# nextpyp/spr_pick

Measured on AMD Instinct MI355X. Metric: train_patches_per_sec, higher is better.
Workload: dtype f32

## Files before the change

spr_pick_amd/csrc/wino.h:

```cpp
#pragma once
#include <hip/hip_runtime.h>

#include "corr.h"

namespace sprk {

bool wino_eligible(const Corr &c);
size_t wino_ws_bytes(const Corr &c);
int wino_conv(const Corr &c, const float *x, const float *x2, const float *w, float *y, float *U, const float *mask,
              int mask_act, hipStream_t s, int unrotB = 0);
bool wino_unrot_eligible(const Corr &c);
bool wino_wgrad_eligible(const sprk_conv_geom &g);
size_t wino_wgrad_ws_bytes(const sprk_conv_geom &g);
int wino_wgrad(const sprk_conv_geom &g, const float *x, const float *x2, const float *gy, float *gw, void *ws,
               sprk_reduce_item *, hipStream_t s);

}
```

spr_pick_amd/csrc/wino.hip:

```cpp
#include <algorithm>
#include <cstdio>
#include <cstdlib>

#include "common.h"
#include "wino.h"
#include "wprep_dev.h"

namespace {

typedef float f32x4 __attribute__((ext_vector_type(4)));
typedef float f32x2 __attribute__((ext_vector_type(2)));
typedef unsigned u32x2 __attribute__((ext_vector_type(2)));
typedef unsigned u32x4 __attribute__((ext_vector_type(4)));
__device__ __forceinline__ unsigned fbits(float v) { return __builtin_bit_cast(unsigned, v); }
typedef __attribute__((address_space(3))) void lds_void;
typedef __amdgpu_buffer_rsrc_t rsrc_t;
constexpr int kXZero = (int)0x80000000;
constexpr float kLeak = 0.1f;

__device__ __forceinline__ rsrc_t make_rsrc(const void *p) {
    return __builtin_amdgcn_make_buffer_rsrc(const_cast<void *>(p), 0, 0x7FFFFFFF, 0x00020000);
}
__device__ __forceinline__ const float *uniform_ptr(const float *p) {
    const unsigned long v = (unsigned long)p;
    const unsigned lo = __builtin_amdgcn_readfirstlane((unsigned)v), hi = __builtin_amdgcn_readfirstlane((unsigned)(v >> 32));
    return (const float *)(((unsigned long)hi << 32) | lo);
}
__device__ __forceinline__ void bdma16(rsrc_t r, int voff, int soff, float *lds_wave_base) {
    __builtin_amdgcn_raw_ptr_buffer_load_lds(r, (lds_void *)lds_wave_base, 16, voff, soff, 0, 0);
}
typedef const __attribute__((address_space(3))) float *lds_cfp;
__device__ __forceinline__ int lds_addr(const void *p) {
    return (int)(unsigned)(__SIZE_TYPE__)(const __attribute__((address_space(3))) char *)p;
}
__device__ __forceinline__ lds_cfp lds_f(int byte_addr) { return (lds_cfp)(__SIZE_TYPE__)(unsigned)byte_addr; }

__device__ __forceinline__ void lds_barrier() {
    asm volatile("s_waitcnt lgkmcnt(0)" ::: "memory");
    __builtin_amdgcn_s_barrier();
    asm volatile("" ::: "memory");
}

__device__ __forceinline__ float act_fn(float v, int act) {
    if (act == SPRK_ACT_LEAKY) return v > 0.f ? v : v * kLeak;
    if (act == SPRK_ACT_RELU) return v > 0.f ? v : 0.f;
    return v;
}

constexpr int CK = sprk::kWinoCK;
template <int SQ>
struct Geo {
    static constexpr int TR = SQ ? 16 : 8, TC = SQ ? 16 : 32;
    static constexpr int RP = TC + 8, RPLANE = (TR + 2) * RP;
    static constexpr int LGTX = SQ ? 3 : 4;
};
constexpr int RAWF = 1792;
static_assert(CK * Geo<0>::RPLANE <= RAWF && CK * Geo<1>::RPLANE <= RAWF, "raw tile fits its stage");
constexpr int ETS = 68;
constexpr int kThreads = 512;
constexpr int kEFloats = 4 * 2 * 32 * ETS;
constexpr int kECFloats = 2 * 96;

__host__ __device__ constexpr int ufloats_of(int NT) { return 16 * NT * CK * 16; }
__host__ __device__ constexpr size_t lds_bytes_of(int NT) {
    return (size_t)(2 * RAWF + 2 * ufloats_of(NT) + kEFloats + kECFloats) * 4;
}

template <int V>
struct IC {
    static constexpr int value = V;
};

#ifdef WINO_STAMP
#define STAMP(k) do { __builtin_amdgcn_sched_barrier(0); if (P == 0) { unsigned long t_; asm volatile("s_memtime %0\n\ts_waitcnt lgkmcnt(0)" : "=s"(t_) :: "memory"); st[(k)] = (unsigned)t_; } __builtin_amdgcn_sched_barrier(0); } while (0)
#else
#define STAMP(k)
#endif
struct KArgs {
    const float *x, *x2, *U, *bias, *scale, *shift, *mask;
    float *y;
    int N, C1, C2, H, W, Cout, padT, padL, act, tilesX, tilesY, ntiles, nc1, nch, up2, xcd, diag, mact;
    int unrotB;
#ifdef WINO_STAMP
    unsigned *dbg;
#endif
};

template <int NT, int SQ, int UNROT = 0>
__global__ __launch_bounds__(kThreads, 1) void wino_conv_kernel(const KArgs a) {
    constexpr int UFLOATS = ufloats_of(NT);
    constexpr int TR = Geo<SQ>::TR, TC = Geo<SQ>::TC, RP = Geo<SQ>::RP, RPLANE = Geo<SQ>::RPLANE, LGTX = Geo<SQ>::LGTX;
    extern __shared__ __attribute__((aligned(16))) float smem[];
    float *Ub = smem;
    float *Rb = smem + 2 * UFLOATS;
    const int tid = threadIdx.x, lane = tid & 63, wave = __builtin_amdgcn_readfirstlane(tid >> 6), l15 = lane & 15,
              lq = lane >> 4;
    const int pg = wave & 3, th = wave >> 2;
    const int grp = blockIdx.y;
    const long HW = (long)a.H * a.W;
    float *EC = smem + 2 * UFLOATS + 2 * RAWF + kEFloats;
    if (tid < NT * 16) {
        const int co = grp * (NT * 16) + tid;
        float sc = 1.f, sh = 0.f;
        if (co < a.Cout) {
            if (a.scale) {
                sc = a.scale[co];
                sh = a.shift[co];
            } else if (a.bias) {
                sh = a.bias[co];
            }
        }
        EC[tid] = sc;
        EC[96 + tid] = sh;
    }

    constexpr int RAWQ = CK * RPLANE / 4;
    int dch = 4, lrow = 0x7000, lcol = 0, loff = 0;
    if (tid < RAWQ) {
        dch = tid / (RPLANE / 4);
        const int rem = tid % (RPLANE / 4);
        lrow = rem / (RP / 4);
        lcol = 4 * (rem % (RP / 4)) - 4;
        loff = (int)(((long)dch * a.H + lrow) * a.W + lcol + 4) * 4;
    }
    int n = 0, by = 0, bx = 0, voff = kXZero;
    auto set_tile = [&](int tile) {
        const int t0 = __builtin_amdgcn_readfirstlane(tile);
        const int q0 = __builtin_amdgcn_readfirstlane(t0 / a.tilesX);
        bx = t0 - q0 * a.tilesX;
        n = __builtin_amdgcn_readfirstlane(q0 / a.tilesY);
        by = q0 - n * a.tilesY;
        const unsigned gy = (unsigned)(by * TR - a.padT + lrow), gx = (unsigned)(bx * TC + lcol);
        voff = (gy < (unsigned)a.H && gx < (unsigned)a.W) ? loff : kXZero;
    };
    const float *rawcur = nullptr, *rawsrc2 = nullptr;
    auto raw_begin = [&]() {
        const long org = (long)(by * TR - a.padT) * a.W + bx * TC - 4;
        rawcur = uniform_ptr(a.x + (long)n * a.C1 * HW + org);
        rawsrc2 = a.C2 > 0 ? uniform_ptr(a.x2 + (long)n * a.C2 * HW + org) : nullptr;
    };
    const int rag1 = (a.C1 % CK) ? a.nc1 - 1 : -1, rag2 = (a.C2 % CK) ? a.nch - 1 : -1;
    auto issue_raw = [&](int c, float *dst, auto ragged) {
        if (c == a.nc1) rawcur = rawsrc2;
        const rsrc_t rs = make_rsrc(rawcur);
        rawcur += (long)CK * HW;
        int vo = voff;
        if constexpr (decltype(ragged)::value != 0)
            if (c == rag1 || c == rag2) vo = dch < (c == rag1 ? a.C1 % CK : a.C2 % CK) ? voff : kXZero;
        if (wave < 7) bdma16(rs, vo, 0, dst + wave * 256);
    };
    const float *Ug = a.U + (long)grp * a.nch * UFLOATS;
    auto issue_u = [&](int c, float *dst) {
        const rsrc_t ur = make_rsrc(Ug + (long)c * UFLOATS);
        constexpr int full = UFLOATS / 2048, rest = UFLOATS % 2048;
#pragma unroll
        for (int gi = 0; gi < full; ++gi) bdma16(ur, tid * 16, gi * 8192, dst + gi * 2048 + wave * 256);
        if (rest && wave < rest / 256) bdma16(ur, tid * 16, full * 8192, dst + full * 2048 + wave * 256);
    };

    f32x4 acc[4][2][NT];

    const int ra = pg == 0 ? 0 : pg == 2 ? 2 : 1, rb = pg == 3 ? 3 : pg == 2 ? 1 : 2;
    const float sgn = pg == 1 ? 1.f : -1.f;
    int rawA[2], rawB[2];
    const int trow0 = (32 * th + l15) >> LGTX, tcol0 = l15 & ((1 << LGTX) - 1);
    constexpr int MTROWS = 16 >> LGTX;
    rawA[0] = lds_addr(Rb + lq * RPLANE + (2 * trow0 + ra) * RP + (4 - a.padL) + 2 * tcol0);
    rawB[0] = lds_addr(Rb + lq * RPLANE + (2 * trow0 + rb) * RP + (4 - a.padL) + 2 * tcol0);
    rawA[1] = rawA[0] + RAWF * 4;
    rawB[1] = rawB[0] + RAWF * 4;
    int bbase = lds_addr(Ub + (4 * pg) * NT * 64 + (NT % 2 == 0 ? 2 * lane : lane));
    asm volatile("" : "+v"(rawA[0]), "+v"(rawA[1]), "+v"(rawB[0]), "+v"(rawB[1]), "+v"(bbase));

    auto transform = [&](auto stage, float (&av)[2][4]) {
        constexpr int S = decltype(stage)::value;
        const lds_cfp pa = lds_f(rawA[S]), pb = lds_f(rawB[S]);
#pragma unroll
        for (int mt = 0; mt < 2; ++mt) {
            float xv[4];
#pragma unroll
            for (int j = 0; j < 4; ++j)
                xv[j] = __builtin_fmaf(pb[mt * 2 * MTROWS * RP + j], sgn, pa[mt * 2 * MTROWS * RP + j]);
            av[mt][0] = xv[0] - xv[2];
            av[mt][1] = xv[1] + xv[2];
            av[mt][2] = xv[2] - xv[1];
            av[mt][3] = xv[1] - xv[3];
        }
    };
    auto mfma12 = [&](const float (&av)[2][4], const float (&bv)[NT], auto pos, auto first) {
        constexpr int p = decltype(pos)::value;
        constexpr bool FIRST = decltype(first)::value != 0;
#pragma unroll
        for (int mt = 0; mt < 2; ++mt)
#pragma unroll
            for (int nt = 0; nt < NT; ++nt) {
                if constexpr (FIRST)
                    acc[p][mt][nt] = __builtin_amdgcn_mfma_f32_16x16x4f32(av[mt][p], bv[nt], (f32x4){0.f, 0.f, 0.f, 0.f}, 0, 0, 0);
                else
                    acc[p][mt][nt] = __builtin_amdgcn_mfma_f32_16x16x4f32(av[mt][p], bv[nt], acc[p][mt][nt], 0, 0, 0);
            }
    };
    auto loadb = [&](float (&bv)[NT], auto stage, auto pos) {
        constexpr int S = decltype(stage)::value, p = decltype(pos)::value;
        if constexpr (NT % 2 == 0) {
            typedef const __attribute__((address_space(3))) f32x2 *lds_cf2p;
#pragma unroll
            for (int q = 0; q < NT / 2; ++q) {
                const f32x2 v = *(lds_cf2p)(__SIZE_TYPE__)(unsigned)(bbase + (S * UFLOATS + (p * (NT / 2) + q) * 128) * 4);
                bv[2 * q] = v[0];
                bv[2 * q + 1] = v[1];
            }
        } else {
            const lds_cfp bp = lds_f(bbase);
#pragma unroll
            for (int nt = 0; nt < NT; ++nt) bv[nt] = bp[S * UFLOATS + (p * NT + nt) * 64];
        }
    };

#ifdef WINO_STAMP
    unsigned st[8] = {}, sv[8] = {};
    if (NT == 6 && a.dbg && blockIdx.x < 4 && lane == 0) {
        a.dbg[(blockIdx.x * 8 + wave) * 16 + 10] = (unsigned)__builtin_amdgcn_s_memtime();
        a.dbg[(blockIdx.x * 8 + wave) * 16 + 11] = (unsigned)__builtin_amdgcn_s_memrealtime();
    }
#endif
    const int nch = a.nch;
    int tile = xcd_slot(blockIdx.x, gridDim.x, a.xcd);
    set_tile(tile);
    auto first_loads = [&]() {
        raw_begin();
        issue_raw(0, Rb, IC<1>{});
        issue_u(0, Ub);
        if (nch > 1) issue_raw(1, Rb + RAWF, IC<1>{});
    };
    first_loads();
    asm volatile("s_waitcnt vmcnt(0)" ::: "memory");
    __syncthreads();
    float aop[2][2][4];
    transform(IC<0>{}, aop[0]);
    __syncthreads();
    auto iter = [&](auto par, int c, auto first, auto checked) {
        constexpr int P = decltype(par)::value;
        constexpr bool CHK = decltype(checked)::value != 0;
        STAMP(0);
        if (!CHK || c + 1 < nch) issue_u(c + 1, Ub + (1 - P) * UFLOATS);
        if (!CHK || c + 2 < nch) issue_raw(c + 2, Rb + P * RAWF, checked);
        STAMP(1);
        float b0[NT], b1[NT];
        if constexpr (NT == 6) {
            transform(IC<1 - P>{}, aop[1 - P]);
            STAMP(2);
            loadb(b0, IC<P>{}, IC<0>{}); mfma12(aop[P], b0, IC<0>{}, first);
            STAMP(3);
            loadb(b0, IC<P>{}, IC<1>{}); mfma12(aop[P], b0, IC<1>{}, first);
            STAMP(4);
            loadb(b0, IC<P>{}, IC<2>{}); mfma12(aop[P], b0, IC<2>{}, first);
            STAMP(5);
            loadb(b0, IC<P>{}, IC<3>{}); mfma12(aop[P], b0, IC<3>{}, first);
            STAMP(6);
            (void)b1;
        } else {
            loadb(b0, IC<P>{}, IC<0>{});
            loadb(b1, IC<P>{}, IC<1>{});
            __builtin_amdgcn_sched_barrier(0);
            mfma12(aop[P], b0, IC<0>{}, first);
            __builtin_amdgcn_sched_barrier(0);
            loadb(b0, IC<P>{}, IC<2>{});
            transform(IC<1 - P>{}, aop[1 - P]);
            __builtin_amdgcn_sched_barrier(0);
            mfma12(aop[P], b1, IC<1>{}, first);
            __builtin_amdgcn_sched_barrier(0);
            loadb(b1, IC<P>{}, IC<3>{});
            __builtin_amdgcn_sched_barrier(0);
            mfma12(aop[P], b0, IC<2>{}, first);
            __builtin_amdgcn_sched_barrier(0);
            mfma12(aop[P], b1, IC<3>{}, first);
        }
        asm volatile("s_waitcnt vmcnt(0)" ::: "memory");
        STAMP(7);
        __syncthreads();
#ifdef WINO_STAMP
        if (c == 10) for (int k = 0; k < 8; ++k) sv[k] = st[k];
#endif
    };
    for (;;) {
        iter(IC<0>{}, 0, IC<1>{}, IC<1>{});
        if (1 < nch) iter(IC<1>{}, 1, IC<0>{}, IC<1>{});
        int c = 2;
        if (rag1 < 0)
            for (; c + 4 < nch; c += 2) {
                iter(IC<0>{}, c, IC<0>{}, IC<0>{});
                iter(IC<1>{}, c + 1, IC<0>{}, IC<0>{});
            }
        for (; c < nch; c += 2) {
            iter(IC<0>{}, c, IC<0>{}, IC<1>{});
            if (c + 1 < nch) iter(IC<1>{}, c + 1, IC<0>{}, IC<1>{});
        }
        const int e_n = n, e_by = by, e_bx = bx;
        const int next = tile + (int)gridDim.x;
        const bool more = next < a.ntiles;
        if (more) {
            set_tile(next);
            first_loads();
        }

    float *E = smem + 2 * UFLOATS + 2 * RAWF;
    const int rl_tx = lane & ((1 << LGTX) - 1), rl_ty = lane >> LGTX;
    int tprime = lane;
    int uoffA = kXZero, uoffB = kXZero, uoffE = kXZero, urot = 0, uk = 0, ub = 0;
    bool uzero = false;
    if constexpr (UNROT) {
        uk = __builtin_amdgcn_readfirstlane(e_n / a.unrotB);
        ub = e_n - uk * a.unrotB;
        urot = (4 - uk) & 3;
        const int P = a.W;
        const int tx = (urot & 1) ? lane >> (6 - LGTX) : rl_tx, ty = (urot & 1) ? lane & ((64 >> LGTX) - 1) : rl_ty;
        tprime = (ty << LGTX) + tx;
        const int s0 = e_by * TR + 2 * ty, v0 = e_bx * TC + 2 * tx;
        const bool top = s0 == 0, last = s0 == P - 2;
        uzero = top;
        if (urot == 0) {
            uoffA = ((s0 + 1) * P + v0) * 4;
            uoffB = last ? kXZero : uoffA + P * 4;
            uoffE = top ? v0 * 4 : kXZero;
        } else if (urot == 2) {
            uoffA = ((P - 2 - s0) * P + (P - 2 - v0)) * 4;
            uoffB = last ? kXZero : uoffA - P * 4;
            uoffE = top ? ((P - 1) * P + (P - 2 - v0)) * 4 : kXZero;
        } else if (urot == 3) {
            uoffA = last ? kXZero : (v0 * P + (P - 3 - s0)) * 4;
            uoffB = last ? kXZero : uoffA + P * 4;
            uoffE = top ? (v0 * P + P - 1) * 4 : last ? (v0 * P) * 4 : kXZero;
        } else {
            uoffA = last ? kXZero : ((P - 1 - v0) * P + s0 + 1) * 4;
            uoffB = last ? kXZero : uoffA - P * 4;
            uoffE = top ? ((P - 2 - v0) * P) * 4 : last ? ((P - 2 - v0) * P + P - 1) * 4 : kXZero;
        }
    }
    const int lane_off = a.up2 ? ((4 * rl_ty) * (2 * a.W) + 4 * rl_tx) * 4 : ((2 * rl_ty) * a.W + 2 * rl_tx) * 4;
    const long tile_org = a.up2 ? ((long)(2 * e_by * TR) * (2 * a.W) + 2 * e_bx * TC) : ((long)(e_by * TR) * a.W + e_bx * TC);
    const long plane = a.up2 ? 4 * HW : HW;
    constexpr int PASSES = (NT + 1) / 2;
    if (!(a.diag & 1))
#pragma unroll
    for (int pass = 0; pass < PASSES; ++pass) {
#pragma unroll
        for (int n2 = 0; n2 < 2; ++n2) {
            const int nt = pass * 2 + n2;
            if (nt < NT) {
#pragma unroll
                for (int mt = 0; mt < 2; ++mt) {
                    const f32x4 s0 = (acc[0][mt][nt] + acc[1][mt][nt]) + acc[2][mt][nt];
                    const f32x4 s1 = (acc[1][mt][nt] - acc[2][mt][nt]) - acc[3][mt][nt];
                    float *e = E + ((pg * 2) * 32 + n2 * 16 + l15) * ETS + 4 * lq + 16 * mt + 32 * th;
                    *reinterpret_cast<f32x4 *>(e) = s0;
                    *reinterpret_cast<f32x4 *>(e + 32 * ETS) = s1;
                }
            }
        }
        lds_barrier();
        auto reader = [&](auto modec) {
            constexpr int MODE = decltype(modec)::value;
            const long ch0 = (MODE == 3 ? (long)(ub * 4 + uk) : (long)e_n) * a.Cout + grp * (NT * 16) + pass * 32 + wave;
            const float *yc = uniform_ptr(a.y + ch0 * plane + (MODE == 3 ? 0 : tile_org));
            const float *mc = MODE == 1 ? uniform_ptr(a.mask + ch0 * plane + tile_org) : nullptr;
#pragma unroll
            for (int it = 0; it < 4; ++it) {
                const int cp = wave + 8 * it;
                const int co = grp * (NT * 16) + pass * 32 + cp;
                if (pass * 32 + cp < NT * 16 && co < a.Cout) {
                    f32x2 mk0 = {1.f, 1.f}, mk1 = {1.f, 1.f};
                    if constexpr (MODE == 1) {
                        const rsrc_t mr = make_rsrc(mc);
                        mk0 = __builtin_bit_cast(f32x2, __builtin_amdgcn_raw_buffer_load_b64(mr, lane_off, 0, 0));
                        mk1 = __builtin_bit_cast(f32x2, __builtin_amdgcn_raw_buffer_load_b64(mr, lane_off, 4 * a.W, 0));
                    }
                    f32x2 s[4];
#pragma unroll
                    for (int w = 0; w < 4; ++w) {
                        s[w][0] = E[((w * 2 + 0) * 32 + cp) * ETS + tprime];
                        s[w][1] = E[((w * 2 + 1) * 32 + cp) * ETS + tprime];
                    }
                    const float sc = EC[pass * 32 + cp], sh = EC[96 + pass * 32 + cp];
                    f32x2 o0 = ((s[0] + s[1]) + s[2]) * sc + sh;
                    f32x2 o1 = ((s[1] - s[2]) - s[3]) * sc + sh;
                    if (a.act == SPRK_ACT_LEAKY) {
                        o0 = __builtin_elementwise_max(o0, o0 * kLeak);
                        o1 = __builtin_elementwise_max(o1, o1 * kLeak);
                    } else if (a.act == SPRK_ACT_RELU) {
                        o0 = __builtin_elementwise_max(o0, (f32x2){0.f, 0.f});
                        o1 = __builtin_elementwise_max(o1, (f32x2){0.f, 0.f});
                    }
                    if constexpr (MODE == 1) {
                        const float neg = a.mact == SPRK_ACT_LEAKY ? kLeak : 0.f;
                        o0[0] *= mk0[0] > 0.f ? 1.f : neg;
                        o0[1] *= mk0[1] > 0.f ? 1.f : neg;
                        o1[0] *= mk1[0] > 0.f ? 1.f : neg;
                        o1[1] *= mk1[1] > 0.f ? 1.f : neg;
                    }
                    const rsrc_t yr = make_rsrc(yc);
                    if constexpr (MODE == 3) {
                        const int rowb = 4 * a.W;
                        if (urot & 1) {
                            const bool rev = urot == 3;
                            __builtin_amdgcn_raw_buffer_store_b64((u32x2){fbits(rev ? o1[0] : o0[0]), fbits(rev ? o0[0] : o1[0])}, yr, uoffA, 0, 0);
                            __builtin_amdgcn_raw_buffer_store_b64((u32x2){fbits(rev ? o1[1] : o0[1]), fbits(rev ? o0[1] : o1[1])}, yr, uoffB, 0, 0);
                            const unsigned e0 = uzero ? 0u : fbits(rev ? o0[0] : o0[1]), e1 = uzero ? 0u : fbits(rev ? o0[1] : o0[0]);
                            __builtin_amdgcn_raw_buffer_store_b32(e0, yr, uoffE, 0, 0);
                            __builtin_amdgcn_raw_buffer_store_b32(e1, yr, uoffE, rowb, 0);
                        } else {
                            const bool rev = urot == 2;
                            __builtin_amdgcn_raw_buffer_store_b64((u32x2){fbits(rev ? o0[1] : o0[0]), fbits(rev ? o0[0] : o0[1])}, yr, uoffA, 0, 0);
                            __builtin_amdgcn_raw_buffer_store_b64((u32x2){fbits(rev ? o1[1] : o1[0]), fbits(rev ? o1[0] : o1[1])}, yr, uoffB, 0, 0);
                            __builtin_amdgcn_raw_buffer_store_b64((u32x2){0u, 0u}, yr, uoffE, 0, 0);
                        }
                    } else if constexpr (MODE == 2) {
                        const int W2b = 8 * a.W;
                        const u32x4 r0 = {fbits(o0[0]), fbits(o0[0]), fbits(o0[1]), fbits(o0[1])},
                                    r1 = {fbits(o1[0]), fbits(o1[0]), fbits(o1[1]), fbits(o1[1])};
                        __builtin_amdgcn_raw_buffer_store_b128(r0, yr, lane_off, 0, 0);
                        __builtin_amdgcn_raw_buffer_store_b128(r0, yr, lane_off, W2b, 0);
                        __builtin_amdgcn_raw_buffer_store_b128(r1, yr, lane_off, 2 * W2b, 0);
                        __builtin_amdgcn_raw_buffer_store_b128(r1, yr, lane_off, 3 * W2b, 0);
                    } else {
                        __builtin_amdgcn_raw_buffer_store_b64((u32x2){fbits(o0[0]), fbits(o0[1])}, yr, lane_off, 0, 0);
                        __builtin_amdgcn_raw_buffer_store_b64((u32x2){fbits(o1[0]), fbits(o1[1])}, yr, lane_off, 4 * a.W, 0);
                    }
                }
                yc += 8 * plane;
                if constexpr (MODE == 1) mc += 8 * plane;
            }
        };
        if constexpr (UNROT)
            reader(IC<3>{});
        else if (a.up2)
            reader(IC<2>{});
        else if (a.mask)
            reader(IC<1>{});
        else
            reader(IC<0>{});
        lds_barrier();
    }
#ifdef WINO_STAMP
        if (NT == 6 && a.dbg && blockIdx.x < 4 && lane == 0) {
            if (tile < (int)gridDim.x) a.dbg[(blockIdx.x * 8 + wave) * 16 + 12] = (unsigned)__builtin_amdgcn_s_memtime();
            a.dbg[(blockIdx.x * 8 + wave) * 16 + 13] = (unsigned)__builtin_amdgcn_s_memtime();
            a.dbg[(blockIdx.x * 8 + wave) * 16 + 14] = (unsigned)__builtin_amdgcn_s_memrealtime();
        }
#endif
        if (!more) break;
        tile = next;
        asm volatile("s_waitcnt vmcnt(0)" ::: "memory");
        __syncthreads();
        transform(IC<0>{}, aop[0]);
        __syncthreads();
    }
}

constexpr int WRH = 4, WRW = 16, WRP = 24;
constexpr int WPB = 4 * 3 * 16 + 4;
constexpr int WAF = 4 * 2048, WSTAGE = 2 * WAF;
constexpr size_t kWgLdsBytes = (size_t)(2 * WSTAGE) * 4;

struct WgKArgs {
    const float *x, *gy;
    float *partial;
    int N, Csrc, cbase, ci0, CinTot, H, W, Cout, padT, padL, regionsX, regionsY, xcd;
};

template <int MT>
__global__ __launch_bounds__(kThreads, 1) void wino_wgrad_kernel(const WgKArgs a) {
    constexpr int PA = 6 * MT * WRP + 4, NA4 = 16 * (PA / 4), NB4 = 32 * (WPB / 4);
    static_assert(16 * PA <= WAF && 32 * WPB <= WAF, "stage holds both operands");
    extern __shared__ __attribute__((aligned(16))) float smem[];
    const int tid = threadIdx.x, lane = tid & 63, wave = __builtin_amdgcn_readfirstlane(tid >> 6), l15 = lane & 15,
              lq = lane >> 4;
    const int pg = wave & 3, h = wave >> 2;
    const int grp = blockIdx.y;
    const int H = a.H, W = a.W;
    const long HW = (long)H * W;
    const int nregions = a.N * a.regionsY * a.regionsX;
    const int c0 = a.cbase + grp * 16 * MT;
    const int have = a.Csrc - c0;

    int offA[4], offB[4], mskA[4];
    {
        const int RY = a.regionsY, RX = a.regionsX;
#pragma unroll
        for (int rd = 0; rd < 4; ++rd) {
            const int q = tid + rd * kThreads;
            const int sl = q / (PA / 4), rem = q % (PA / 4);
            const int row = rem / (6 * MT), mt = (rem % (6 * MT)) / 6, c4 = rem % 6;
            const bool va = q < NA4 && rem < 36 * MT && 16 * mt + sl < have;
            offA[rd] = va ? (int)(((16 * mt + sl) * HW + (long)row * W + 4 * c4) * 4) : kXZero;
            int m = 0;
#pragma unroll
            for (int yt = 0; yt < 4; ++yt) {
                const int ry = yt == 0 ? 0 : yt == 1 ? 1 : yt == 2 ? RY - 1 : 0;
                const bool rok = (unsigned)(ry * WRH - a.padT + row) < (unsigned)H;
#pragma unroll
                for (int xt = 0; xt < 4; ++xt) {
                    const int rx = xt == 0 ? 0 : xt == 1 ? 1 : xt == 2 ? RX - 1 : 0;
                    const bool cok = (unsigned)(rx * WRW - 4 + 4 * c4) < (unsigned)W;
                    m |= (rok && cok) ? 1 << (4 * yt + xt) : 0;
                }
            }
            mskA[rd] = va ? m : 0;
            const int sb = q / (WPB / 4), remb = q % (WPB / 4);
            const int rowb = remb / 12, ntb = (remb % 12) / 4, c4b = remb % 4;
            const int chb = (sb >> 4) * 48 + 16 * ntb + (sb & 15);
            offB[rd] = (q < NB4 && remb < 48 && chb < a.Cout) ? (int)((chb * HW + (long)rowb * W + 4 * c4b) * 4) : kXZero;
        }
    }
    int cur_rx, cur_ry, cur_n, d_rx, d_ry, d_n;
    {
        const int r0 = xcd_slot(blockIdx.x, gridDim.x, a.xcd);
        const int q0 = r0 / a.regionsX;
        cur_rx = __builtin_amdgcn_readfirstlane(r0 - q0 * a.regionsX);
        cur_n = __builtin_amdgcn_readfirstlane(q0 / a.regionsY);
        cur_ry = __builtin_amdgcn_readfirstlane(q0 - (q0 / a.regionsY) * a.regionsY);
        const int st = gridDim.x, t0 = st / a.regionsX;
        d_rx = __builtin_amdgcn_readfirstlane(st - t0 * a.regionsX);
        d_n = __builtin_amdgcn_readfirstlane(t0 / a.regionsY);
        d_ry = __builtin_amdgcn_readfirstlane(t0 - (t0 / a.regionsY) * a.regionsY);
// ... 144 lines not shown
    }
    };
    if (zmix) {
        regions(IC<1>{});
        finish();
    } else {
        regions(IC<0>{});
        finish();
    }
}

struct WgRanges {
    int end[4], parts[4];
};
__global__ __launch_bounds__(256) void wino_wgrad_reduce_kernel(const float *__restrict__ partial, float *__restrict__ gw,
                                                                long n, int CinTot, WgRanges rg) {
    __shared__ float red[8][33];
    const int el = threadIdx.x & 31, sl = threadIdx.x >> 5;
    const long e = (long)blockIdx.x * 32 + el;
    float s = 0.f;
    if (e < n) {
        const int ci = (int)((e / 9) % CinTot);
        int parts = rg.parts[3];
#pragma unroll
        for (int i = 2; i >= 0; --i)
            if (ci < rg.end[i]) parts = rg.parts[i];
        float s0 = 0.f, s1 = 0.f;
        int p = sl;
        for (; p + 8 < parts; p += 16) {
            s0 += partial[(long)p * n + e];
            s1 += partial[(long)(p + 8) * n + e];
        }
        if (p < parts) s0 += partial[(long)p * n + e];
        s = s0 + s1;
    }
    red[sl][el] = s;
    __syncthreads();
    if (sl == 0 && e < n) {
        float t = red[0][el];
#pragma unroll
        for (int j = 1; j < 8; ++j) t += red[j][el];
        gw[e] = t;
    }
}

bool wg_split(int C, int *g48, int *tail) {
    *g48 = C / 48;
    *tail = C % 48;
    return *tail <= 16;
}

int nt_of(int Cout) { return Cout <= 48 ? 3 : 6; }

int wino_square(int H, int W) {
    if (H % Geo<0>::TR == 0 && W % Geo<0>::TC == 0) return 0;
    if (H % Geo<1>::TR == 0 && W % Geo<1>::TC == 0) return 1;
    return -1;
}

}

namespace sprk {

constexpr int kClassWino = 3;

bool wino_eligible(const Corr &g) {
    static const int on = knob_env("SPRK_WINO", 1);
    if (!on) return false;
    if (g.KH != 3 || g.KW != 3 || g.stride != 1 || g.dil != 1 || g.up1 || g.mfma_only || g.ep.res) return false;
    if (g.Hout != g.Hin || g.Wout != g.Win) return false;
    const int H = g.Hin, W = g.Win;
    const int sq = wino_square(H, W);
    if (sq < 0) return false;
    const int TR = sq ? Geo<1>::TR : Geo<0>::TR, TC = sq ? Geo<1>::TC : Geo<0>::TC;
    if (g.padL < 0 || g.padL > 4 || g.padT < 0) return false;
    if (g.C1 < 1 || g.C2 < 0 || g.Cout < 33) return false;
    const int NT = nt_of(g.Cout), groups = cdiv(g.Cout, NT * 16);
    if ((double)g.Cout / (groups * NT * 16) < 0.7) return false;
    if (!g.pin() && (long)g.N * (H / TR) * (W / TC) * groups < 128) return false;
    if ((long)4 * H * W * 4 >= 0x7FFFFFFFL) return false;
    return true;
}

size_t wino_ws_bytes(const Corr &c) {
    const int NT = nt_of(c.Cout), groups = cdiv(c.Cout, NT * 16), nch = cdiv(c.C1, CK) + cdiv(c.C2, CK);
    return (size_t)groups * nch * ufloats_of(NT) * sizeof(float);
}

bool wino_unrot_eligible(const Corr &c) {
    return wino_eligible(c) && nt_of(c.Cout) == 6 && c.Hin == 64 && c.Win == 64 && c.N % 4 == 0 && !c.ep.up2 && c.taps == 0;
}

int wino_conv(const Corr &w, const float *x, const float *x2, const float *taps, float *y, float *U, const float *mask,
              int mask_act, hipStream_t s, int unrotB) {
    const int NT = nt_of(w.Cout), groups = cdiv(w.Cout, NT * 16);
    const int kclass = w.Cout > 48 ? kClassWino : 2;
    KArgs a{};
    a.x = x; a.x2 = x2; a.U = U; a.bias = w.ep.bias; a.scale = w.ep.scale; a.shift = w.ep.shift; a.y = y;
    a.N = w.N; a.C1 = w.C1; a.C2 = w.C2; a.H = w.Hin; a.W = w.Win; a.Cout = w.Cout; a.padT = w.padT; a.padL = w.padL;
    a.act = w.ep.act;
    a.up2 = w.ep.up2 ? 1 : 0;
    a.mask = a.up2 ? nullptr : mask;
    a.mact = mask_act;
    a.xcd = xcd_on();
    static const int diag = sprk::diag_env("SPRK_WINO_DIAG");
    a.diag = diag;
    a.unrotB = unrotB;
    if (unrotB && (mask || !wino_unrot_eligible(w) || unrotB * 4 != w.N)) {
        set_error("wino_conv: no un-rotated store for this call");
        return SPRK_EINVAL;
    }
    static const int unrot_sq = knob_env("SPRK_WINO_UNROT_SQ", 0);
    const int sq = (unrotB && unrot_sq) ? 1 : wino_square(a.H, a.W);
    a.tilesX = a.W / (sq ? Geo<1>::TC : Geo<0>::TC); a.tilesY = a.H / (sq ? Geo<1>::TR : Geo<0>::TR);
    a.ntiles = a.tilesX * a.tilesY * w.N;
    a.nc1 = cdiv(w.C1, CK);
    a.nch = a.nc1 + cdiv(w.C2, CK);
    if ((((uintptr_t)x | (uintptr_t)x2 | (uintptr_t)y | (uintptr_t)U) & 15) != 0) {
        set_error("wino_conv: tensors must be 16-byte aligned");
        return SPRK_EINVAL;
    }
    const long total = (long)groups * a.nch * NT * CK * 16;
    if (int rc = wprep_site(wprep_item(WPREP_WINO, taps, U, total, {w.Cout, w.C1, w.C2, a.nc1, a.nch, NT, groups, w.taps}), s))
        return rc;
    static const int persist = knob_env("SPRK_WINO_PERSIST", 1);
    const dim3 grid(persist ? std::min(a.ntiles, std::max(1, num_cus() / groups)) : a.ntiles, groups);
    const size_t lds = lds_bytes_of(NT);
    auto launch = [&](auto kernel) {
        if (int rc = lds_optin(kernel, lds, "wino_conv")) return rc;
        hipLaunchKernelGGL(kernel, grid, dim3(kThreads), lds, s, a);
        return (int)SPRK_OK;
    };
#ifdef WINO_STAMP
    static unsigned *dbg = nullptr;
    static int dumped = 0;
    if (!dbg) { hipMalloc(&dbg, 4 * 8 * 16 * 4); hipMemset(dbg, 0, 4 * 8 * 16 * 4); }
    a.dbg = dbg;
#endif
    prof_begin(kclass, w.flops, s);
    if (int rc = unrotB ? (sq ? launch(wino_conv_kernel<6, 1, 1>) : launch(wino_conv_kernel<6, 0, 1>))
                 : NT == 6 ? (sq ? launch(wino_conv_kernel<6, 1>) : launch(wino_conv_kernel<6, 0>))
                         : (sq ? launch(wino_conv_kernel<3, 1>) : launch(wino_conv_kernel<3, 0>)))
        return rc;
    prof_end(kclass, s);
#ifdef WINO_STAMP
    if (NT == 6 && !sq && ++dumped == 5 && getenv("SPRK_WINO_STAMP")) {
        hipDeviceSynchronize();
        unsigned h[4 * 8 * 16];
        hipMemcpy(h, dbg, sizeof h, hipMemcpyDeviceToHost);
        FILE *f = fopen(getenv("SPRK_WINO_STAMP"), "a");
        for (int wg = 0; wg < 4; ++wg)
            for (int wv = 0; wv < 8; ++wv) {
                fprintf(f, "wg%d w%d", wg, wv);
                for (int k = 0; k < 16; ++k) fprintf(f, " %u", h[(wg * 8 + wv) * 16 + k]);
                fprintf(f, "\n");
            }
        fclose(f);
    }
#endif
    g_wino_launches.fetch_add(1, std::memory_order_relaxed);
    return SPRK_OK;
}

bool wino_wgrad_eligible(const sprk_conv_geom &g) {
    static const int on = knob_env("SPRK_WINO_WGRAD", 1);
    if (!on) return false;
    if (g.KH != 3 || g.KW != 3 || g.stride != 1 || g.dil != 1 || g.up1) return false;
    const int H = g.Hin, W = g.Win, padT = g.pad_top, padL = g.pad_left;
    if (g.Hout != H || g.Wout != W || H % WRH || W % WRW) return false;
    if (padL < 0 || padL > 4 || padT < 0 || padT > 4) return false;
    if (g.Cout < 81 || g.Cout > 96) return false;
    int g48, tail;
    if (g.C1 < 1 || !wg_split(g.C1, &g48, &tail)) return false;
    if (g.C2 > 0 && !wg_split(g.C2, &g48, &tail)) return false;
    static const long min_regions = knob_env("SPRK_WINO_WGRAD_MIN", 0);
    const bool has_tail = (g.C1 % 48) != 0 || (g.C2 % 48) != 0;
    const long need = min_regions > 0 ? min_regions : (has_tail ? 8192 : 2048);
    if ((long)g.N * (H / WRH) * (W / WRW) < need) return false;
    if ((long)48 * H * W * 4 >= 0x7FFFFFFFL || (long)g.Cout * H * W * 4 >= 0x7FFFFFFFL) return false;
    return true;
}

constexpr int kWgParts = 256;
constexpr int kClassWinoW = 4;

size_t wino_wgrad_ws_bytes(const sprk_conv_geom &g) {
    return (size_t)kWgParts * g.Cout * (g.C1 + g.C2) * 9 * sizeof(float);
}

int wino_wgrad(const sprk_conv_geom &g, const float *x, const float *x2, const float *gy, float *gw, void *ws,
               sprk_reduce_item *, hipStream_t s) {
    float *partial = (float *)ws;
    if ((((uintptr_t)x | (uintptr_t)x2 | (uintptr_t)gy | (uintptr_t)partial) & 15) != 0) {
        set_error("wino_wgrad: tensors must be 16-byte aligned");
        return SPRK_EINVAL;
    }
    const double flops = conv_flops(g);
    const int CinTot = g.C1 + g.C2;
    WgRanges rg{};
    int nr = 0;
    auto launch = [&](const float *src, int Csrc, int ci0) -> int {
        int g48, tail;
        wg_split(Csrc, &g48, &tail);
        WgKArgs a{src, gy, partial, g.N, Csrc, 0, ci0, CinTot, g.Hin, g.Win, g.Cout, g.pad_top, g.pad_left, g.Win / WRW,
                  g.Hin / WRH, xcd_on()};
        if (g48 > 0) {
            if (int rc = lds_optin(wino_wgrad_kernel<3>, kWgLdsBytes, "wino_wgrad")) return rc;
            const int parts = std::min(kWgParts, num_cus()) / g48;
            prof_begin(kClassWinoW, flops * (48.0 * g48) / CinTot, s);
            hipLaunchKernelGGL(wino_wgrad_kernel<3>, dim3(parts, g48), dim3(kThreads), kWgLdsBytes, s, a);
            prof_end(kClassWinoW, s);
            if (int rc = check_launch("wino_wgrad<3>")) return rc;
            rg.end[nr] = ci0 + 48 * g48;
            rg.parts[nr++] = parts;
        }
        if (tail > 0) {
            if (int rc = lds_optin(wino_wgrad_kernel<1>, kWgLdsBytes, "wino_wgrad")) return rc;
            WgKArgs t = a;
            t.cbase = 48 * g48;
            prof_begin(kClassWinoW, flops * (double)tail / CinTot, s);
            hipLaunchKernelGGL(wino_wgrad_kernel<1>, dim3(std::min(kWgParts, num_cus()), 1), dim3(kThreads), kWgLdsBytes, s, t);
            prof_end(kClassWinoW, s);
            if (int rc = check_launch("wino_wgrad<1>")) return rc;
            rg.end[nr] = ci0 + Csrc;
            rg.parts[nr++] = std::min(kWgParts, num_cus());
        }
        return SPRK_OK;
    };
    if (int rc = launch(x, g.C1, 0)) return rc;
    if (g.C2 > 0)
        if (int rc = launch(x2, g.C2, g.C1)) return rc;
    for (int i = nr; i < 4; ++i) rg.end[i] = CinTot, rg.parts[i] = rg.parts[nr - 1];
    const long n = (long)g.Cout * CinTot * 9;
    hipLaunchKernelGGL(wino_wgrad_reduce_kernel, dim3(cdiv(n, 32)), dim3(256), 0, s, partial, gw, n, CinTot, rg);
    if (int rc = check_launch("wino_wgrad_reduce")) return rc;
    g_wino_launches.fetch_add(1, std::memory_order_relaxed);
    return SPRK_OK;
}

}
```

Measured before the change: 1981.

## Specialize Winograd epilogue by form and share buffer descriptors across channels

The output epilogue of the Winograd conv kernel is restructured into compile-time specialized variants keyed by a host-computed form code that covers store mode, activation/affine kind and shared-descriptor use. This removes per-channel runtime activation branches and buffer resource rebuilds. When the planes fit in the 32-bit buffer range, a single descriptor is reused with a scalar channel offset. Tile index decode also switches from per-tile divisions to incremental advancement, and the inverse-transform adds are split into half-vectors. Each form becomes its own specialized copy of the epilogue, which increases code size and adds a dispatch switch; a new ISA counting script is also added.

After: 1979. No clear change (-0.1%).

```diff
diff --git a/profiles/isa_count.py b/profiles/isa_count.py
--- /dev/null
+++ b/profiles/isa_count.py
@@ -0,0 +1,104 @@
+#!/usr/bin/env python3
+import argparse
+import re
+import sys
+
+CLASSES = ["mfma", "valu", "pk", "scalar", "lds_rd", "lds_wr", "buf_ld", "buf_st", "wait", "barrier", "other"]
+
+
+def classify(m):
+    if m.startswith(("v_mfma", "v_smfmac")):
+        return "mfma"
+    if m.startswith("v_pk_"):
+        return "pk"
+    if m.startswith("v_"):
+        return "valu"
+    if m.startswith("s_waitcnt"):
+        return "wait"
+    if m.startswith("s_barrier"):
+        return "barrier"
+    if m.startswith("s_"):
+        return "scalar"
+    if m.startswith(("ds_read", "ds_load")):
+        return "lds_rd"
+    if m.startswith(("ds_write", "ds_store")):
+        return "lds_wr"
+    if m.startswith("buffer_load"):
+        return "buf_ld"
+    if m.startswith("buffer_store"):
+        return "buf_st"
+    return "other"
+
+
+LABEL = re.compile(r"^([A-Za-z_.$][\w.$]*):")
+INSN = re.compile(r"^\s+([a-z][a-z0-9_]*)\b(.*)$")
+
+
+def kernels(lines):
+    names = [m.group(1) for ln in lines if (m := re.match(r"^\s*\.amdhsa_kernel\s+(\S+)", ln))]
+    out = {}
+    for name in names:
+        start = next((i for i, ln in enumerate(lines) if ln.startswith(name + ":")), None)
+        if start is None:
+            continue
+        end = next((i for i in range(start, len(lines)) if lines[i].startswith(".Lfunc_end")), len(lines))
+        out[name] = (start + 1, end)
+    return out
+
+
+def blocks(lines, lo, hi):
+    out = [("<entry>", dict.fromkeys(CLASSES, 0), [])]
+    for ln in lines[lo:hi]:
+        code = ln.split(";")[0].rstrip()
+        if not code:
+            continue
+        if m := LABEL.match(code):
+            out.append((m.group(1), dict.fromkeys(CLASSES, 0), []))
+            continue
+        m = INSN.match(code)
+        if not m or code.lstrip().startswith("."):
+            continue
+        mnem, rest = m.group(1), m.group(2)
+        out[-1][1][classify(mnem)] += 1
+        if mnem.startswith(("s_cbranch", "s_branch", "s_endpgm", "s_setpc")):
+            out[-1][2].append(rest.strip())
+            base, _, k = out[-1][0].partition("+")
+            out.append(("%s+%d" % (base, int(k or 0) + 1), dict.fromkeys(CLASSES, 0), []))
+    return out
+
+
+def main():
+    ap = argparse.ArgumentParser(description=__doc__, formatter_class=argparse.RawDescriptionHelpFormatter)
+    ap.add_argument("asm", help="assembly of one source (hipcc ... --cuda-device-only -S)")
+    ap.add_argument("kernel", nargs="?", help="substring of the kernel's symbol")
+    ap.add_argument("--list", action="store_true", help="print the kernel symbols and their instruction totals")
+    args = ap.parse_args()
+    with open(args.asm) as f:
+        lines = f.read().split("\n")
+    ks = kernels(lines)
+    if args.list or not args.kernel:
+        for name, (lo, hi) in ks.items():
+            print("%6d  %s" % (sum(sum(c.values()) for _, c, _ in blocks(lines, lo, hi)), name))
+        return 0
+    hits = [k for k in ks if args.kernel in k]
+    if len(hits) != 1:
+        print("kernel %r matches %d symbols: %s" % (args.kernel, len(hits), hits), file=sys.stderr)
+        return 2
+    lo, hi = ks[hits[0]]
+    bl = blocks(lines, lo, hi)
+    print("# %s" % hits[0])
+    print("%-16s" % "block" + "".join("%8s" % c for c in CLASSES) + "%8s  %s" % ("non-mfma", "branches to"))
+    total = dict.fromkeys(CLASSES, 0)
+    for label, cnt, br in bl:
+        n = sum(cnt.values())
+        if n == 0:
+            continue
+        for c in CLASSES:
+            total[c] += cnt[c]
+        print("%-16s" % label + "".join("%8d" % cnt[c] for c in CLASSES) + "%8d  %s" % (n - cnt["mfma"], " ".join(br)))
+    print("%-16s" % "total" + "".join("%8d" % total[c] for c in CLASSES) + "%8d" % (sum(total.values()) - total["mfma"]))
+    return 0
+
+
+if __name__ == "__main__":
+    sys.exit(main())
diff --git a/spr_pick_amd/csrc/wino.h b/spr_pick_amd/csrc/wino.h
--- a/spr_pick_amd/csrc/wino.h
+++ b/spr_pick_amd/csrc/wino.h
@@ -10,6 +10,7 @@
 int wino_conv(const Corr &c, const float *x, const float *x2, const float *w, float *y, float *U, const float *mask,
               int mask_act, hipStream_t s, int unrotB = 0);
 bool wino_unrot_eligible(const Corr &c);
+bool wino_shared_desc_fits(long H, long W, bool up2);
 bool wino_wgrad_eligible(const sprk_conv_geom &g);
 size_t wino_wgrad_ws_bytes(const sprk_conv_geom &g);
 int wino_wgrad(const sprk_conv_geom &g, const float *x, const float *x2, const float *gy, float *gw, void *ws,
diff --git a/spr_pick_amd/csrc/wino.hip b/spr_pick_amd/csrc/wino.hip
--- a/spr_pick_amd/csrc/wino.hip
+++ b/spr_pick_amd/csrc/wino.hip
@@ -13,6 +13,8 @@
 typedef unsigned u32x2 __attribute__((ext_vector_type(2)));
 typedef unsigned u32x4 __attribute__((ext_vector_type(4)));
 __device__ __forceinline__ unsigned fbits(float v) { return __builtin_bit_cast(unsigned, v); }
+__device__ __forceinline__ f32x2 lo_half(f32x4 v) { return __builtin_shufflevector(v, v, 0, 1); }
+__device__ __forceinline__ f32x2 hi_half(f32x4 v) { return __builtin_shufflevector(v, v, 2, 3); }
 typedef __attribute__((address_space(3))) void lds_void;
 typedef __amdgpu_buffer_rsrc_t rsrc_t;
 constexpr int kXZero = (int)0x80000000;
@@ -81,6 +83,8 @@
     float *y;
     int N, C1, C2, H, W, Cout, padT, padL, act, tilesX, tilesY, ntiles, nc1, nch, up2, xcd, diag, mact;
     int unrotB;
+    int form;
+    int chstep;
 #ifdef WINO_STAMP
     unsigned *dbg;
 #endif
@@ -124,12 +128,31 @@
         loff = (int)(((long)dch * a.H + lrow) * a.W + lcol + 4) * 4;
     }
     int n = 0, by = 0, bx = 0, voff = kXZero;
-    auto set_tile = [&](int tile) {
-        const int t0 = __builtin_amdgcn_readfirstlane(tile);
-        const int q0 = __builtin_amdgcn_readfirstlane(t0 / a.tilesX);
-        bx = t0 - q0 * a.tilesX;
-        n = __builtin_amdgcn_readfirstlane(q0 / a.tilesY);
-        by = q0 - n * a.tilesY;
+    int cur_bx, cur_by, cur_n, d_bx, d_by, d_n;
+    {
+        const int t0 = xcd_slot(blockIdx.x, gridDim.x, a.xcd);
+        const int q0 = t0 / a.tilesX;
+        cur_bx = __builtin_amdgcn_readfirstlane(t0 - q0 * a.tilesX);
+        cur_n = __builtin_amdgcn_readfirstlane(q0 / a.tilesY);
+        cur_by = __builtin_amdgcn_readfirstlane(q0 - (q0 / a.tilesY) * a.tilesY);
+        const int st = gridDim.x, s0 = st / a.tilesX;
+        d_bx = __builtin_amdgcn_readfirstlane(st - s0 * a.tilesX);
+        d_n = __builtin_amdgcn_readfirstlane(s0 / a.tilesY);
+        d_by = __builtin_amdgcn_readfirstlane(s0 - (s0 / a.tilesY) * a.tilesY);
+    }
+    auto advance_tile = [&]() {
+        cur_bx += d_bx;
+        const int cx = cur_bx >= a.tilesX;
+        cur_bx -= cx ? a.tilesX : 0;
+        cur_by += d_by + cx;
+        const int cy = cur_by >= a.tilesY;
+        cur_by -= cy ? a.tilesY : 0;
+        cur_n += d_n + cy;
+    };
+    auto set_tile = [&]() {
+        bx = cur_bx;
+        by = cur_by;
+        n = cur_n;
         const unsigned gy = (unsigned)(by * TR - a.padT + lrow), gx = (unsigned)(bx * TC + lcol);
         voff = (gy < (unsigned)a.H && gx < (unsigned)a.W) ? loff : kXZero;
     };
@@ -226,7 +249,7 @@
 #endif
     const int nch = a.nch;
     int tile = xcd_slot(blockIdx.x, gridDim.x, a.xcd);
-    set_tile(tile);
+    set_tile();
     auto first_loads = [&]() {
         raw_begin();
         issue_raw(0, Rb, IC<1>{});
@@ -300,7 +323,8 @@
         const int next = tile + (int)gridDim.x;
         const bool more = next < a.ntiles;
         if (more) {
-            set_tile(next);
+            advance_tile();
+            set_tile();
             first_loads();
         }
 
@@ -340,18 +364,31 @@
     const int lane_off = a.up2 ? ((4 * rl_ty) * (2 * a.W) + 4 * rl_tx) * 4 : ((2 * rl_ty) * a.W + 2 * rl_tx) * 4;
     const long tile_org = a.up2 ? ((long)(2 * e_by * TR) * (2 * a.W) + 2 * e_bx * TC) : ((long)(e_by * TR) * a.W + e_bx * TC);
     const long plane = a.up2 ? 4 * HW : HW;
+    int lo0 = lane_off;
+    asm volatile("" : "+v"(lo0));
+    const int rstep = a.up2 ? 8 * a.W : 4 * a.W;
+    const int lo1 = lo0 + rstep, lo2 = lo0 + 2 * rstep, lo3 = lo0 + 3 * rstep;
+    const int uoffE1 = uoffE + 4 * a.W;
+    int ebase0 = lds_addr(E + wave * ETS + tprime), ebase1 = ebase0 + 8 * ETS * 4, ecbase = lds_addr(EC + wave);
+    asm volatile("" : "+v"(ebase0), "+v"(ebase1), "+v"(ecbase));
+    int lim = a.Cout - grp * (NT * 16) - wave;
+    asm volatile("" : "+s"(lim));
     constexpr int PASSES = (NT + 1) / 2;
-    if (!(a.diag & 1))
-#pragma unroll
-    for (int pass = 0; pass < PASSES; ++pass) {
+    auto do_pass = [&](auto passc) {
+        constexpr int pass = decltype(passc)::value;
+        constexpr int ITS = (NT * 16 - pass * 32) >= 32 ? 4 : (NT * 16 - pass * 32) / 8;
+        int form = a.form;
+        asm volatile("" : "+s"(form));
 #pragma unroll
         for (int n2 = 0; n2 < 2; ++n2) {
             const int nt = pass * 2 + n2;
             if (nt < NT) {
 #pragma unroll
                 for (int mt = 0; mt < 2; ++mt) {
-                    const f32x4 s0 = (acc[0][mt][nt] + acc[1][mt][nt]) + acc[2][mt][nt];
-                    const f32x4 s1 = (acc[1][mt][nt] - acc[2][mt][nt]) - acc[3][mt][nt];
+                    const f32x4 a0 = acc[0][mt][nt], a1 = acc[1][mt][nt], a2 = acc[2][mt][nt], a3 = acc[3][mt][nt];
+                    const f32x2 s0l = (lo_half(a0) + lo_half(a1)) + lo_half(a2), s0h = (hi_half(a0) + hi_half(a1)) + hi_half(a2);
+                    const f32x2 s1l = (lo_half(a1) - lo_half(a2)) - lo_half(a3), s1h = (hi_half(a1) - hi_half(a2)) - hi_half(a3);
+                    const f32x4 s0 = __builtin_shufflevector(s0l, s0h, 0, 1, 2, 3), s1 = __builtin_shufflevector(s1l, s1h, 0, 1, 2, 3);
                     float *e = E + ((pg * 2) * 32 + n2 * 16 + l15) * ETS + 4 * lq + 16 * mt + 32 * th;
                     *reinterpret_cast<f32x4 *>(e) = s0;
                     *reinterpret_cast<f32x4 *>(e + 32 * ETS) = s1;
@@ -359,87 +396,113 @@
             }
         }
         lds_barrier();
-        auto reader = [&](auto modec) {
+        auto reader = [&](auto modec, auto epc, auto sharedc) {
             constexpr int MODE = decltype(modec)::value;
+            constexpr int EP = decltype(epc)::value;
+            constexpr bool SHARED = decltype(sharedc)::value != 0;
             const long ch0 = (MODE == 3 ? (long)(ub * 4 + uk) : (long)e_n) * a.Cout + grp * (NT * 16) + pass * 32 + wave;
             const float *yc = uniform_ptr(a.y + ch0 * plane + (MODE == 3 ? 0 : tile_org));
             const float *mc = MODE == 1 ? uniform_ptr(a.mask + ch0 * plane + tile_org) : nullptr;
-#pragma unroll
-            for (int it = 0; it < 4; ++it) {
-                const int cp = wave + 8 * it;
-                const int co = grp * (NT * 16) + pass * 32 + cp;
-                if (pass * 32 + cp < NT * 16 && co < a.Cout) {
-                    f32x2 mk0 = {1.f, 1.f}, mk1 = {1.f, 1.f};
-                    if constexpr (MODE == 1) {
-                        const rsrc_t mr = make_rsrc(mc);
-                        mk0 = __builtin_bit_cast(f32x2, __builtin_amdgcn_raw_buffer_load_b64(mr, lane_off, 0, 0));
-                        mk1 = __builtin_bit_cast(f32x2, __builtin_amdgcn_raw_buffer_load_b64(mr, lane_off, 4 * a.W, 0));
+            const rsrc_t yr0 = make_rsrc(yc), mr0 = make_rsrc(MODE == 1 ? mc : yc);
+            int ur = urot;
+            asm volatile("" : "+s"(ur));
+            auto channel = [&](auto itc) {
+                constexpr int it = decltype(itc)::value;
+                const int cq = pass * 32 + 8 * it;
+                const rsrc_t yr = SHARED ? yr0 : make_rsrc(yc + it * 8 * plane),
+                             mr = SHARED || MODE != 1 ? mr0 : make_rsrc(mc + it * 8 * plane);
+                const int so = SHARED ? it * a.chstep : 0;
+                f32x2 mk0 = {1.f, 1.f}, mk1 = {1.f, 1.f};
+                if constexpr (MODE == 1) {
+                    mk0 = __builtin_bit_cast(f32x2, __builtin_amdgcn_raw_buffer_load_b64(mr, lo0, so, 0));
+                    mk1 = __builtin_bit_cast(f32x2, __builtin_amdgcn_raw_buffer_load_b64(mr, lo1, so, 0));
+                }
+                const lds_cfp ep = lds_f((it & 1) ? ebase1 : ebase0);
+                const int eo = (it >> 1) * 16 * ETS;
+                f32x2 s[4];
+#pragma unroll
+                for (int w = 0; w < 4; ++w) {
+                    s[w][0] = ep[(w * 2 + 0) * 32 * ETS + eo];
+                    s[w][1] = ep[(w * 2 + 1) * 32 * ETS + eo];
+                }
+                f32x2 o0, o1;
+                if constexpr (EP == 0) {
+                    o0 = ((s[0] + s[1]) + s[2]) + 0.f;
+                    o1 = ((s[1] - s[2]) - s[3]) + 0.f;
+                } else {
+                    const float sc = lds_f(ecbase)[cq], sh = lds_f(ecbase)[96 + cq];
+                    o0 = ((s[0] + s[1]) + s[2]) * sc + sh;
+                    o1 = ((s[1] - s[2]) - s[3]) * sc + sh;
+                }
+                if constexpr (EP == 2) {
+                    o0 = __builtin_elementwise_max(o0, o0 * kLeak);
+                    o1 = __builtin_elementwise_max(o1, o1 * kLeak);
+                } else if constexpr (EP == 3) {
+                    o0 = __builtin_elementwise_max(o0, (f32x2){0.f, 0.f});
+                    o1 = __builtin_elementwise_max(o1, (f32x2){0.f, 0.f});
+                }
+                if constexpr (MODE == 1) {
+                    const float neg = a.mact == SPRK_ACT_LEAKY ? kLeak : 0.f;
+                    o0[0] *= mk0[0] > 0.f ? 1.f : neg;
+                    o0[1] *= mk0[1] > 0.f ? 1.f : neg;
+                    o1[0] *= mk1[0] > 0.f ? 1.f : neg;
+                    o1[1] *= mk1[1] > 0.f ? 1.f : neg;
+                }
+                if constexpr (MODE == 3) {
+                    if (ur & 1) {
+                        const bool rev = ur == 3;
+                        __builtin_amdgcn_raw_buffer_store_b64((u32x2){fbits(rev ? o1[0] : o0[0]), fbits(rev ? o0[0] : o1[0])}, yr, uoffA, so, 0);
+                        __builtin_amdgcn_raw_buffer_store_b64((u32x2){fbits(rev ? o1[1] : o0[1]), fbits(rev ? o0[1] : o1[1])}, yr, uoffB, so, 0);
+                        const unsigned e0 = uzero ? 0u : fbits(rev ? o0[0] : o0[1]), e1 = uzero ? 0u : fbits(rev ? o0[1] : o0[0]);
+                        __builtin_amdgcn_raw_buffer_store_b32(e0, yr, uoffE, so, 0);
+                        __builtin_amdgcn_raw_buffer_store_b32(e1, yr, uoffE1, so, 0);
+                    } else {
+                        const bool rev = ur == 2;
+                        __builtin_amdgcn_raw_buffer_store_b64((u32x2){fbits(rev ? o0[1] : o0[0]), fbits(rev ? o0[0] : o0[1])}, yr, uoffA, so, 0);
+                        __builtin_amdgcn_raw_buffer_store_b64((u32x2){fbits(rev ? o1[1] : o1[0]), fbits(rev ? o1[0] : o1[1])}, yr, uoffB, so, 0);
+                        __builtin_amdgcn_raw_buffer_store_b64((u32x2){0u, 0u}, yr, uoffE, so, 0);
                     }
-                    f32x2 s[4];
-#pragma unroll
-                    for (int w = 0; w < 4; ++w) {
-                        s[w][0] = E[((w * 2 + 0) * 32 + cp) * ETS + tprime];
-                        s[w][1] = E[((w * 2 + 1) * 32 + cp) * ETS + tprime];
-                    }
-                    const float sc = EC[pass * 32 + cp], sh = EC[96 + pass * 32 + cp];
-                    f32x2 o0 = ((s[0] + s[1]) + s[2]) * sc + sh;
-                    f32x2 o1 = ((s[1] - s[2]) - s[3]) * sc + sh;
-                    if (a.act == SPRK_ACT_LEAKY) {
-                        o0 = __builtin_elementwise_max(o0, o0 * kLeak);
-                        o1 = __builtin_elementwise_max(o1, o1 * kLeak);
-                    } else if (a.act == SPRK_ACT_RELU) {
-                        o0 = __builtin_elementwise_max(o0, (f32x2){0.f, 0.f});
-                        o1 = __builtin_elementwise_max(o1, (f32x2){0.f, 0.f});
-                    }
-                    if constexpr (MODE == 1) {
-                        const float neg = a.mact == SPRK_ACT_LEAKY ? kLeak : 0.f;
-                        o0[0] *= mk0[0] > 0.f ? 1.f : neg;
-                        o0[1] *= mk0[1] > 0.f ? 1.f : neg;
-                        o1[0] *= mk1[0] > 0.f ? 1.f : neg;
-                        o1[1] *= mk1[1] > 0.f ? 1.f : neg;
-                    }
-                    const rsrc_t yr = make_rsrc(yc);
-                    if constexpr (MODE == 3) {
-                        const int rowb = 4 * a.W;
-                        if (urot & 1) {
-                            const bool rev = urot == 3;
-                            __builtin_amdgcn_raw_buffer_store_b64((u32x2){fbits(rev ? o1[0] : o0[0]), fbits(rev ? o0[0] : o1[0])}, yr, uoffA, 0, 0);
-                            __builtin_amdgcn_raw_buffer_store_b64((u32x2){fbits(rev ? o1[1] : o0[1]), fbits(rev ? o0[1] : o1[1])}, yr, uoffB, 0, 0);
-                            const unsigned e0 = uzero ? 0u : fbits(rev ? o0[0] : o0[1]), e1 = uzero ? 0u : fbits(rev ? o0[1] : o0[0]);
-                            __builtin_amdgcn_raw_buffer_store_b32(e0, yr, uoffE, 0, 0);
-                            __builtin_amdgcn_raw_buffer_store_b32(e1, yr, uoffE, rowb, 0);
-                        } else {
-                            const bool rev = urot == 2;
-                            __builtin_amdgcn_raw_buffer_store_b64((u32x2){fbits(rev ? o0[1] : o0[0]), fbits(rev ? o0[0] : o0[1])}, yr, uoffA, 0, 0);
-                            __builtin_amdgcn_raw_buffer_store_b64((u32x2){fbits(rev ? o1[1] : o1[0]), fbits(rev ? o1[0] : o1[1])}, yr, uoffB, 0, 0);
-                            __builtin_amdgcn_raw_buffer_store_b64((u32x2){0u, 0u}, yr, uoffE, 0, 0);
-                        }
-                    } else if constexpr (MODE == 2) {
-                        const int W2b = 8 * a.W;
-                        const u32x4 r0 = {fbits(o0[0]), fbits(o0[0]), fbits(o0[1]), fbits(o0[1])},
-                                    r1 = {fbits(o1[0]), fbits(o1[0]), fbits(o1[1]), fbits(o1[1])};
-                        __builtin_amdgcn_raw_buffer_store_b128(r0, yr, lane_off, 0, 0);
-                        __builtin_amdgcn_raw_buffer_store_b128(r0, yr, lane_off, W2b, 0);
-                        __builtin_amdgcn_raw_buffer_store_b128(r1, yr, lane_off, 2 * W2b, 0);
-                        __builtin_amdgcn_raw_buffer_store_b128(r1, yr, lane_off, 3 * W2b, 0);
-                    } else {
-                        __builtin_amdgcn_raw_buffer_store_b64((u32x2){fbits(o0[0]), fbits(o0[1])}, yr, lane_off, 0, 0);
-                        __builtin_amdgcn_raw_buffer_store_b64((u32x2){fbits(o1[0]), fbits(o1[1])}, yr, lane_off, 4 * a.W, 0);
-                    }
+                } else if constexpr (MODE == 2) {
+                    const u32x4 r0 = {fbits(o0[0]), fbits(o0[0]), fbits(o0[1]), fbits(o0[1])},
+                                r1 = {fbits(o1[0]), fbits(o1[0]), fbits(o1[1]), fbits(o1[1])};
+                    __builtin_amdgcn_raw_buffer_store_b128(r0, yr, lo0, so, 0);
+                    __builtin_amdgcn_raw_buffer_store_b128(r0, yr, lo1, so, 0);
+                    __builtin_amdgcn_raw_buffer_store_b128(r1, yr, lo2, so, 0);
+                    __builtin_amdgcn_raw_buffer_store_b128(r1, yr, lo3, so, 0);
+                } else {
+                    __builtin_amdgcn_raw_buffer_store_b64((u32x2){fbits(o0[0]), fbits(o0[1])}, yr, lo0, so, 0);
+                    __builtin_amdgcn_raw_buffer_store_b64((u32x2){fbits(o1[0]), fbits(o1[1])}, yr, lo1, so, 0);
                 }
-                yc += 8 * plane;
-                if constexpr (MODE == 1) mc += 8 * plane;
+            };
+            if (__builtin_expect(pass * 32 + 8 * (ITS - 1) < lim, 1)) {
+                channel(IC<0>{});
+                if constexpr (ITS > 1) channel(IC<1>{});
+                if constexpr (ITS > 2) channel(IC<2>{});
+                if constexpr (ITS > 3) channel(IC<3>{});
+            } else {
+                if (pass * 32 < lim) channel(IC<0>{});
+                if constexpr (ITS > 1) if (pass * 32 + 8 < lim) channel(IC<1>{});
+                if constexpr (ITS > 2) if (pass * 32 + 16 < lim) channel(IC<2>{});
+                if constexpr (ITS > 3) if (pass * 32 + 24 < lim) channel(IC<3>{});
             }
         };
-        if constexpr (UNROT)
-            reader(IC<3>{});
-        else if (a.up2)
-            reader(IC<2>{});
-        else if (a.mask)
-            reader(IC<1>{});
-        else
-            reader(IC<0>{});
+#define WINO_READER(m, e, sh) case ((m) * 4 + (e)) * 2 + (sh): reader(IC<m>{}, IC<e>{}, IC<sh>{}); break;
+#define WINO_READERS(m, sh) WINO_READER(m, 0, sh) WINO_READER(m, 1, sh) WINO_READER(m, 2, sh) WINO_READER(m, 3, sh)
+        if constexpr (UNROT) {
+            switch (form) { WINO_READERS(3, 1) }
+        } else {
+            switch (form) {
+                WINO_READERS(0, 0) WINO_READERS(0, 1) WINO_READERS(1, 0) WINO_READERS(1, 1) WINO_READERS(2, 0) WINO_READERS(2, 1)
+            }
+        }
+#undef WINO_READERS
+#undef WINO_READER
         lds_barrier();
+    };
+    if (!(a.diag & 1)) {
+        do_pass(IC<0>{});
+        do_pass(IC<1>{});
+        if constexpr (PASSES > 2) do_pass(IC<2>{});
     }
 #ifdef WINO_STAMP
         if (NT == 6 && a.dbg && blockIdx.x < 4 && lane == 0) {
@@ -750,6 +813,11 @@
     return true;
 }
 
+bool wino_shared_desc_fits(long H, long W, bool up2) {
+    const long plane_bytes = (up2 ? 4 : 1) * H * W * 4;
+    return H > 0 && W > 0 && (3 * 8 + 1) * plane_bytes <= 0x7FFFFFFFL;
+}
+
 size_t wino_ws_bytes(const Corr &c) {
     const int NT = nt_of(c.Cout), groups = cdiv(c.Cout, NT * 16), nch = cdiv(c.C1, CK) + cdiv(c.C2, CK);
     return (size_t)groups * nch * ufloats_of(NT) * sizeof(float);
@@ -774,6 +842,10 @@
     static const int diag = sprk::diag_env("SPRK_WINO_DIAG");
     a.diag = diag;
     a.unrotB = unrotB;
+    const int epk = (!a.scale && !a.bias && a.act != SPRK_ACT_LEAKY && a.act != SPRK_ACT_RELU) ? 0
+                    : a.act == SPRK_ACT_LEAKY ? 2 : a.act == SPRK_ACT_RELU ? 3 : 1;
+    a.chstep = wino_shared_desc_fits(a.H, a.W, a.up2 != 0) ? (int)(8 * (a.up2 ? 4L : 1L) * a.H * a.W * 4) : 0;
+    a.form = ((unrotB ? 3 : a.up2 ? 2 : a.mask ? 1 : 0) * 4 + epk) * 2 + (a.chstep ? 1 : 0);
     if (unrotB && (mask || !wino_unrot_eligible(w) || unrotB * 4 != w.N)) {
         set_error("wino_conv: no un-rotated store for this call");
         return SPRK_EINVAL;
@@ -907,3 +979,5 @@
 }
 
 }
+
+extern "C" int sprk_wino_shared_desc_fits(long H, long W, int up2) { return sprk::wino_shared_desc_fits(H, W, up2 != 0) ? 1 : 0; }
```
